# GenomicBreeding/GenomicBreedingModels.jl

Hardware: AMD Instinct MI355X
Metric: GRM+GBLUP genotype-cells/s (n x p) (higher is better)
Workload: dtype f64

## Files before the change

### genomicbreedingmodels.jl_amd/csrc/gbm_internal.h

```cpp
#pragma once
#include <hip/hip_runtime.h>
#include <stdint.h>
#include <functional>
#include <string>
#include <vector>

#include "../../include/gbm.h"

namespace gbm {

constexpr int64_t kNPadTile = 128;
constexpr int64_t kRhsRows = 64;
constexpr int kCholNB = 64;

inline int64_t round_up(int64_t x, int64_t m) { return (x + m - 1) / m * m; }
inline int64_t npad_of(int64_t n) { return round_up(n < 1 ? 1 : n, kNPadTile); }
inline int64_t gdim_of(int64_t n) { return npad_of(n) + kRhsRows; }

void set_error(const std::string& msg);
int fail(int code, const std::string& msg);
const std::string& last_error();

const char* knob(const char* name);
int64_t knob_i64(const char* name, int64_t def);

#define GBM_HIP_TRY(expr)                                                                      \
  do {                                                                                         \
    hipError_t e_ = (expr);                                                                    \
    if (e_ != hipSuccess)                                                                      \
      return ::gbm::fail(GBM_E_HIP, std::string("HIP error '") + hipGetErrorString(e_) +       \
                                        "' at " __FILE__ ":" + std::to_string(__LINE__) + " (" #expr ")"); \
  } while (0)

#define GBM_LAUNCH_CHECK() GBM_HIP_TRY(hipGetLastError())

#define GBM_TRY(expr)              \
  do {                             \
    int rc_ = (expr);              \
    if (rc_ != GBM_OK) return rc_; \
  } while (0)

int launch_grm(const double* Zt, int64_t ldz, int64_t p, int64_t n, double* G, int64_t ldg,
               void* ws, int64_t ws_bytes, hipStream_t s, int accum = 0, int32_t* err_out = nullptr);
bool grm_can_accumulate(int64_t n, int64_t p);
int launch_standardize_rows(const double* Xt, int64_t ldx, int64_t p, int64_t n, double* Zt, int64_t ldz, double* mean,
                            double* sd, int32_t* keep, int64_t* q_dev, hipStream_t s, bool beside_tiles = false);
bool standardize_fits_beside_tiles(int64_t n);
int64_t grm_workspace_bytes(int64_t n, int64_t p);
int launch_grm_export(const double* G, int64_t ldg, int64_t n, double inv_q, double* out, int64_t ldo, hipStream_t s);
int launch_predict(const double* Xt, int64_t ldx, int64_t p, int64_t n, const double* b, int64_t ldb, int64_t nrhs,
                   double* partial, int64_t nchunks, double* out, int64_t ldo, hipStream_t s);
int64_t predict_chunks(int64_t n, int64_t p);
int launch_add_inplace(double* a, const double* b, int64_t n, hipStream_t s);
int launch_standardize_i8(const int8_t* D, int64_t ldd, int64_t p, int64_t n, int ploidy, double* Zt, int64_t ldz,
                          double* mean, double* sd, int32_t* keep, int64_t* q_dev, hipStream_t s);
int launch_marker_rows(const double* Zt, int64_t ldz, int64_t p, int64_t n, const double* A, int64_t lda, int64_t nrhs,
                       double inv_q, const int64_t* q_dev, const double* sd, const int32_t* keep, double* B,
                       int64_t ldb, hipStream_t s);
int launch_marker_rows_i8(const int8_t* D, int64_t ldd, int64_t p, int64_t n, int ploidy, const double* A, int64_t lda,
                          int64_t nrhs, double inv_q, const int64_t* q_dev, const double* mean, const double* sd,
                          const int32_t* keep, double* B, int64_t ldb, hipStream_t s);
int launch_grm_exact(const int8_t* D, int64_t ldd, int64_t p, int64_t n, int ploidy, double* G, int64_t ldg,
                     double* mean, double* sd, int32_t* keep, int64_t* q_dev, int accum, void* ws, int64_t ws_bytes,
                     int32_t* slices_out, hipStream_t s);
int grm_exact_status(const void* ws, int64_t n, int64_t p, hipStream_t s);
int launch_gather_dosage(const double* Xt, int64_t ldx, int64_t p, const int32_t* idx, int64_t nT, int8_t* D,
                         hipStream_t s);
int launch_dosage_from_f64(const double* X, int64_t ldx, int64_t n, int64_t p, int8_t* D, int64_t ldd, int32_t* bad,
                           hipStream_t s);
// ... 79 lines not shown
```

### genomicbreedingmodels.jl_amd/csrc/grm.hip

```cpp
#include <algorithm>
#include <atomic>
#include <cmath>
#include <cstdio>
#include <cstdlib>
#include <map>
#include <mutex>
#include <queue>
#include <tuple>
#include <vector>

#include "chol_device.h"

namespace gbm {

constexpr int BT = 128;
constexpr int BK = 16;
constexpr int WPS = 2;
constexpr int LROW = BT + 2;
constexpr int STAGE = 2 * BK * LROW;

__device__ __forceinline__ void tile_of(int64_t t, int64_t& ti, int64_t& tj) {
  int64_t r = (int64_t)((sqrt(8.0 * (double)t + 1.0) - 1.0) * 0.5);
  while ((r + 1) * (r + 2) / 2 <= t) r++;
  while (r * (r + 1) / 2 > t) r--;
// ... 200 lines not shown
#pragma unroll
      for (int q = 0; q < ET; q++) b[st][q] = kv ? row[sb.e0 + q * 16 + fc] : 0.0;
    }
#pragma unroll
    for (int st = 0; st < 4; st++)
#pragma unroll
      for (int q = 0; q < ET; q++)
#pragma unroll
        for (int m = 0; m < 4; m++) acc[m][q] = __builtin_amdgcn_mfma_f64_16x16x4f64(a[st][m], b[st][q], acc[m][q], 0, 0, 0);
  }
  const int64_t rows = (int64_t)sb.erb * 256;
  constexpr int w = 16 * ET;
#pragma unroll
  for (int m = 0; m < 4; m++)
#pragma unroll
    for (int q = 0; q < ET; q++)
#pragma unroll
      for (int r = 0; r < 4; r++)
        part[((int64_t)ks * rows + i0 + m * 16 + fr + 4 * r) * w + q * 16 + fc] = acc[m][q][r];
}

template <int ET>
__global__ void __launch_bounds__(256, ET == 1 ? 4 : 1) grm_edge_kernel(const double* __restrict__ U, int64_t ldu, int64_t K,
                                                       SliceBounds sb, double* __restrict__ part) {
  grm_edge_pass<ET>(U, ldu, K, sb, blockIdx.x, part, threadIdx.x & 63, threadIdx.x >> 6);
}

__global__ void __launch_bounds__(256) grm_edge_reduce_kernel(const double* __restrict__ part, int64_t n,
                                                              SliceBounds sb, double* __restrict__ G, int64_t ldg,
                                                              int accum) {
  const int64_t idx = (int64_t)blockIdx.x * 256 + threadIdx.x;
  if (idx >= n * sb.er) return;
  const int64_t i = idx / sb.er;
  const int c = (int)(idx - i * sb.er);
  const int64_t rows = (int64_t)sb.erb * 256;
  const int w = 16 * sb.et;
  double acc = 0.0;
  for (int s = 0; s < sb.es; s++) acc += part[((int64_t)s * rows + i) * w + c];
  double* g = G + i * ldg + sb.e0 + c;
  *g = accum ? *g + acc : acc;
}

template <int MODE>
__global__ void __launch_bounds__(256, WPS)
syrk_kernel(const double* __restrict__ U, int64_t ldu, int64_t K, int64_t c0, int64_t lim,
            double* __restrict__ C, int64_t ldc, double* __restrict__ slab, int64_t ntiles, SliceBounds sb,
            double* __restrict__ Ld, double* __restrict__ Dinv, int32_t* __restrict__ info, int64_t fk0,
// ... 620 lines not shown
    const int64_t ti1 = (std::min(row_hi, gdim) - k1 + BT - 1) / BT;
    if (ti1 <= own.ti0) return GBM_OK;
    const int64_t m = ti1 - own.ti0;
    syrk_kernel<kSub><<<dim3((unsigned)m, (unsigned)(own.ncols + own.rhs)), 256, 0, s>>>(
        G + k0 * ldg, ldg, nb, k1, lim, G, ldg, nullptr, 0, SliceBounds{}, Ld, Dinv, info, -1, own);
    GBM_LAUNCH_CHECK();
    return GBM_OK;
  }
  if (nb == 64 && lim <= chol_small_lim()) {
    const int64_t m = (lim + 63) / 64;
    syrk64_sub_kernel<false><<<(unsigned)(m * (m + 1) / 2), 256, 0, s>>>(G + k0 * ldg, ldg, k1, lim, G, ldg, Ld, Dinv, info,
                                                                  next_k0, 0, (int)(nb / 64), ColKeep{});
    GBM_LAUNCH_CHECK();
    return GBM_OK;
  }
  const int64_t m = (lim + BT - 1) / BT;
  const int64_t ntiles = m * (m + 1) / 2;
  syrk_kernel<kSub><<<(unsigned)ntiles, 256, 0, s>>>(G + k0 * ldg, ldg, nb, k1, lim, G, ldg, nullptr, ntiles, SliceBounds{}, Ld,
                                                     Dinv, info, next_k0, own);
  GBM_LAUNCH_CHECK();
  return GBM_OK;
}

struct AuxStream {
  hipStream_t s = nullptr;
  hipEvent_t fork = nullptr, join = nullptr;
  ~AuxStream() {
    if (fork) (void)hipEventDestroy(fork);
    if (join) (void)hipEventDestroy(join);
  }
};
static int aux_stream(hipStream_t caller, AuxStream& a, bool* usable) {
  *usable = false;
  int dev = 0;
  GBM_HIP_TRY(hipGetDevice(&dev));
  if (caller) {
    int sdev = -1;
    if (hipStreamGetDevice(caller, &sdev) != hipSuccess) {
      (void)hipGetLastError();
      return GBM_OK;
    }
    if (sdev != dev) return GBM_OK;
  }
  static std::mutex mu;
  static std::map<int, hipStream_t> streams;
  {
    std::lock_guard<std::mutex> lock(mu);
    hipStream_t& hs = streams[dev];
    if (!hs) GBM_HIP_TRY(hipStreamCreateWithFlags(&hs, hipStreamNonBlocking));
    a.s = hs;
  }
  GBM_HIP_TRY(hipEventCreateWithFlags(&a.fork, hipEventDisableTiming));
  GBM_HIP_TRY(hipEventCreateWithFlags(&a.join, hipEventDisableTiming));
  *usable = true;
  return GBM_OK;
}

static int64_t grm_second_doubles(const GrmPlan& g) {
  return (g.persist && !g.sb.fuse && g.sb.n >= 2) ? g.tile_elems : 0;
}
static int64_t grm_counter_doubles(const GrmPlan& g) {
  return grm_second_doubles(g) + 4 + (g.sb.fuse ? (g.ntiles + 1) / 2 : 0);
}
int64_t grm_workspace_bytes(int64_t n, int64_t p) {
  const GrmPlan g = plan(n, p);
  return (g.main_doubles + g.edge_doubles + grm_counter_doubles(g)) * (int64_t)sizeof(double);
}

static int check_grm_args(const double* Zt, int64_t ldz, int64_t p, int64_t n, double* G, int64_t ldg) {
  const int64_t npad = npad_of(n);
  if (!Zt || !G || p < 1 || n < 1 || ldz < npad || ldg < npad || (ldz & 1) || (ldg & 1))
    return fail(GBM_E_ARG, "gbm_dev_grm: bad arguments (need ldz, ldg >= npad(n), both even)");
  if (((uintptr_t)Zt & 15) != 0 || ((uintptr_t)G & 15) != 0)
    return fail(GBM_E_ARG, "gbm_dev_grm: Zt and G must be 16-byte aligned");
  return GBM_OK;
}

static int launch_persist(const GrmPlan& g, SliceBounds sb, int s0, int cnt, const double* Zt, int64_t ldz, int64_t p,
                          int64_t lim, double* G, int64_t ldg, void* ws, int32_t* ctr, hipStream_t s) {
  sb.s0 = s0;
  sb.cnt = cnt;
  const int64_t units = (int64_t)cnt * g.ntiles;
  const unsigned pgrid = (unsigned)(units < resident_wgs() ? units : resident_wgs());
  if (g.sb.fuse)
    syrk_kernel<kPersistFused><<<pgrid, 256, 0, s>>>(Zt, ldz, p, 0, lim, G, ldg, (double*)ws, g.ntiles, sb, nullptr,
                                                     nullptr, ctr, -1, TileOwner{});
  else
    syrk_kernel<kPersist><<<pgrid, 256, 0, s>>>(Zt, ldz, p, 0, lim, G, ldg, (double*)ws, g.ntiles, sb, nullptr,
                                                nullptr, ctr, -1, TileOwner{});
  GBM_LAUNCH_CHECK();
  return GBM_OK;
}

static int launch_grm_edge(const GrmPlan& g, const double* Zt, int64_t ldz, int64_t p, int64_t n, double* G,
                           int64_t ldg, void* ws, int accum, hipStream_t es) {
  const unsigned eg = (unsigned)((int64_t)g.sb.erb * g.sb.es);
  double* part = (double*)ws + g.sb.eslab_off;
  switch (g.sb.et) {
    case 1: grm_edge_kernel<1><<<eg, 256, 0, es>>>(Zt, ldz, p, g.sb, part); break;
    case 2: grm_edge_kernel<2><<<eg, 256, 0, es>>>(Zt, ldz, p, g.sb, part); break;
    case 3: grm_edge_kernel<3><<<eg, 256, 0, es>>>(Zt, ldz, p, g.sb, part); break;
    default: grm_edge_kernel<4><<<eg, 256, 0, es>>>(Zt, ldz, p, g.sb, part); break;
  }
  GBM_LAUNCH_CHECK();
  if (g.edge_concurrent) {
    grm_edge_reduce_kernel<<<(unsigned)((n * g.sb.er + 255) / 256), 256, 0, es>>>(part, n, g.sb, G, ldg, accum);
    GBM_LAUNCH_CHECK();
  }
  return GBM_OK;
}

int launch_grm_syrk(const double* Zt, int64_t ldz, int64_t p, int64_t n, double* G, int64_t ldg, void* ws,
                    int64_t ws_bytes, hipStream_t s, int accum = 0) {
  int rc = check_grm_args(Zt, ldz, p, n, G, ldg);
  if (rc != GBM_OK) return rc;
  const GrmPlan g = plan(n, p);
  SliceBounds sb = g.sb;
  sb.accum = accum;
  const int64_t need = (g.main_doubles + g.edge_doubles + grm_counter_doubles(g)) * (int64_t)sizeof(double);
  if (need > 0 && (!ws || ws_bytes < need))
    return fail(GBM_E_ARG, "gbm_dev_grm: workspace too small (" + std::to_string(ws_bytes) + " < " +
                               std::to_string(need) + ")");
  const unsigned grid = (unsigned)(g.sb.n * ((g.ntiles + 7) & ~(int64_t)7));
  if (g.sb.carry) GBM_HIP_TRY(hipMemsetAsync(ws, 0, (size_t)(g.ntiles + 1) * sizeof(int32_t), s));
  int32_t* ctr = reinterpret_cast<int32_t*>((double*)ws + g.main_doubles + g.edge_doubles + grm_second_doubles(g));
// ... 10 lines not shown
      GBM_HIP_TRY(hipStreamWaitEvent(ax->s, ax->fork, 0));
    }
  }
  if (g.persist) {
    GBM_HIP_TRY(hipMemsetAsync(ctr, 0, (size_t)(8 + (g.sb.fuse ? g.ntiles : 0)) * sizeof(int32_t), s));
    rc = launch_persist(g, sb, 0, g.sb.n, Zt, ldz, p, lim, G, ldg, ws, ctr, s);
    if (rc != GBM_OK) return rc;
  } else {
    syrk_kernel<kSplit><<<grid, 256, 0, s>>>(Zt, ldz, p, 0, lim, G, ldg, (double*)ws, g.ntiles, sb, nullptr, nullptr,
                                             nullptr, -1, TileOwner{});
    GBM_LAUNCH_CHECK();
  }
  if (g.sb.er > 0) {
    rc = launch_grm_edge(g, Zt, ldz, p, n, G, ldg, ws, accum, ax ? ax->s : s);
    if (rc != GBM_OK) return rc;
    if (ax) {
      GBM_HIP_TRY(hipEventRecord(ax->join, ax->s));
      GBM_HIP_TRY(hipStreamWaitEvent(s, ax->join, 0));
    }
  }
  return GBM_OK;
}

int launch_standardize_grm_syrk(const double* X, int64_t ldx, int64_t p, int64_t n, double* Zt, int64_t ldz,
                                double* mean, double* sd, int32_t* keep, int64_t* q, double* G, int64_t ldg, void* ws,
                                int64_t ws_bytes, hipStream_t s) {
  int rc = check_grm_args(Zt, ldz, p, n, G, ldg);
  if (rc != GBM_OK) return rc;
  if (!X || !mean || !sd || !keep || !q || ldx < n || (X == Zt && ldx != ldz))
    return fail(GBM_E_ARG, "gbm_dev_standardize_grm_syrk: bad arguments");
  const GrmPlan g = plan(n, p);
  const int64_t h = g.sb.n >= 2 ? std::min<int64_t>(p, (int64_t)BK * g.sb.b[1]) : p;
  AuxStream aux;
  bool overlap = knob_i64("GBM_GRM_STD_OVERLAP", 1) != 0 && g.persist && !g.sb.fuse && g.sb.n >= 2 && h < p &&
                 standardize_fits_beside_tiles(n);
  if (overlap) {
    rc = aux_stream(s, aux, &overlap);
    if (rc != GBM_OK) return rc;
  }
  if (!overlap) {
    rc = launch_standardize_rows(X, ldx, p, n, Zt, ldz, mean, sd, keep, q, s);
    if (rc != GBM_OK) return rc;
    return launch_grm_syrk(Zt, ldz, p, n, G, ldg, ws, ws_bytes, s);
  }
  const int64_t need = (g.main_doubles + g.edge_doubles + grm_counter_doubles(g)) * (int64_t)sizeof(double);
  if (!ws || ws_bytes < need)
    return fail(GBM_E_ARG, "gbm_dev_standardize_grm_syrk: workspace too small (" + std::to_string(ws_bytes) + " < " +
                               std::to_string(need) + ")");
  int32_t* ctr = reinterpret_cast<int32_t*>((double*)ws + g.main_doubles + g.edge_doubles + grm_second_doubles(g)) - 8;
  const int64_t lim = g.sb.er > 0 ? g.sb.e0 : n;
  GBM_TRY(launch_standardize_rows(X, ldx, h, n, Zt, ldz, mean, sd, keep, q, s));
  GBM_HIP_TRY(hipMemsetAsync(ctr, 0, 16 * sizeof(int32_t), s));
  GBM_HIP_TRY(hipEventRecord(aux.fork, s));
  GBM_HIP_TRY(hipStreamWaitEvent(aux.s, aux.fork, 0));
  GBM_TRY(launch_persist(g, g.sb, 0, 1, Zt, ldz, p, lim, G, ldg, ws, ctr + 8, s));
  GBM_TRY(launch_standardize_rows(X + h * ldx, ldx, p - h, n, Zt + h * ldz, ldz, mean + h, sd + h, keep + h, q, aux.s,
                                  true));
  if (g.sb.er > 0) GBM_TRY(launch_grm_edge(g, Zt, ldz, p, n, G, ldg, ws, 0, aux.s));
  GBM_TRY(launch_persist(g, g.sb, 1, g.sb.n - 1, Zt, ldz, p, lim, G, ldg, ws, ctr, aux.s));
  GBM_HIP_TRY(hipEventRecord(aux.join, aux.s));
  GBM_HIP_TRY(hipStreamWaitEvent(s, aux.join, 0));
  return GBM_OK;
}

int launch_grm_reduce(int64_t n, int64_t p, double* G, int64_t ldg, const void* ws, hipStream_t s, int accum = 0,
                      int32_t* err_out = nullptr) {
  const GrmPlan g = plan(n, p);
  if (g.sb.n == 1 && g.sb.er == 0) return GBM_OK;
  if (!ws) return fail(GBM_E_ARG, "gbm_dev_grm_reduce: workspace required");
  if (g.sb.er > 0 && !g.edge_concurrent) {
    grm_edge_reduce_kernel<<<(unsigned)((n * g.sb.er + 255) / 256), 256, 0, s>>>((const double*)ws + g.sb.eslab_off, n,
                                                                                 g.sb, G, ldg, accum);
    GBM_LAUNCH_CHECK();
  }
  if (g.sb.n == 1 || g.sb.fuse) return GBM_OK;
  if (g.sb.carry && err_out) {
    GBM_HIP_TRY(hipMemcpyAsync(err_out, (const int32_t*)ws + g.ntiles, sizeof(int32_t), hipMemcpyDeviceToDevice, s));
    return GBM_OK;
  }
  if (g.sb.carry) {
    int32_t err = 0;
    GBM_HIP_TRY(hipMemcpyAsync(&err, (const int32_t*)ws + g.ntiles, sizeof(int32_t), hipMemcpyDeviceToHost, s));
    GBM_HIP_TRY(hipStreamSynchronize(s));
    if (err < 0)
// ... 75 lines not shown
}

extern "C" int gbm_dev_grm_syrk(const double* Zt, int64_t ldz, int64_t p, int64_t n, double* G, int64_t ldg,
                                void* workspace, int64_t ws_bytes, void* stream) {
  return gbm::launch_grm_syrk(Zt, ldz, p, n, G, ldg, workspace, ws_bytes, (hipStream_t)stream);
}

extern "C" int gbm_dev_standardize_grm_syrk(const double* Xt, int64_t ldx, int64_t p, int64_t n, double* Zt, int64_t ldz,
                                            double* mean, double* sd, int32_t* keep, int64_t* q_dev, double* G,
                                            int64_t ldg, void* workspace, int64_t ws_bytes, void* stream) {
  return gbm::launch_standardize_grm_syrk(Xt, ldx, p, n, Zt, ldz, mean, sd, keep, q_dev, G, ldg, workspace, ws_bytes,
                                          (hipStream_t)stream);
}

extern "C" int gbm_dev_grm_reduce(int64_t n, int64_t p, double* G, int64_t ldg, const void* workspace, void* stream) {
  if (!G || n < 1 || p < 1 || ldg < gbm::npad_of(n)) return gbm::fail(GBM_E_ARG, "gbm_dev_grm_reduce: bad arguments");
  return gbm::launch_grm_reduce(n, p, G, ldg, workspace, (hipStream_t)stream);
}

extern "C" int gbm_dev_grm_slices(int64_t n, int64_t p) {
  return gbm::plan(n, p).sb.n;
}

namespace gbm {
__global__ void __launch_bounds__(256) add_inplace_kernel(double* __restrict__ a, const double* __restrict__ b,
                                                          int64_t n) {
  for (int64_t i = ((int64_t)blockIdx.x * 256 + threadIdx.x) * 2; i < n; i += (int64_t)gridDim.x * 512) {
    if (i + 1 < n) {
      double2 x = *reinterpret_cast<const double2*>(a + i);
      const double2 y = *reinterpret_cast<const double2*>(b + i);
      x.x += y.x;
      x.y += y.y;
      *reinterpret_cast<double2*>(a + i) = x;
    } else {
      a[i] += b[i];
    }
  }
}

int launch_add_inplace(double* a, const double* b, int64_t n, hipStream_t s) {
  if (n <= 0) return GBM_OK;
  const int64_t want = (n + 511) / 512;
  add_inplace_kernel<<<(unsigned)(want < 8192 ? want : 8192), 256, 0, s>>>(a, b, n);
  GBM_LAUNCH_CHECK();
  return GBM_OK;
}
// ... 15 lines not shown
```

### genomicbreedingmodels.jl_amd/csrc/stats.hip

```cpp
#include <type_traits>

#include "counter_hash.h"
#include "gbm_internal.h"

namespace gbm {

__global__ void __launch_bounds__(256) synth_kernel(double* __restrict__ Xt, int64_t ldx, int64_t p,
                                                    int64_t n, uint64_t seed, int64_t j0) {
  for (int64_t j = blockIdx.y; j < p; j += gridDim.y) {
    const uint64_t base = mix64(seed * 0xD1B54A32D192ED03ull + (uint64_t)(j0 + j));
    const uint64_t thr = 214748364ull + (((base >> 32) * 1932735283ull) >> 32);
    double* row = Xt + j * ldx;
    for (int64_t i = (int64_t)blockIdx.x * 1024 + threadIdx.x; i < (int64_t)(blockIdx.x + 1) * 1024 && i < ldx;
         i += 256) {
      double v = 0.0;
      if (i < n) {
        const uint64_t h = mix64(base ^ ((uint64_t)i * 0x8CB92BA72F3D8DD7ull));
        const int d = ((h & 0xFFFFFFFFull) < thr) + ((h >> 32) < thr);
        v = 0.5 * (double)d;
      }
      row[i] = v;
    }
  }
}
// ... 43 lines not shown
  return (double)d * xs;
}

#ifndef GBM_STD_NT
#define GBM_STD_NT 1
#endif
template <typename T>
__device__ __forceinline__ double load_x(const T* row, int64_t i, double xs) {
  if constexpr (std::is_same<T, int8_t>::value)
    return dosage_x(row[i], xs);
  else if constexpr (GBM_STD_NT == 1 || GBM_STD_NT == 2)
    return __builtin_nontemporal_load(row + i);
  else
    return row[i];
}
__device__ __forceinline__ void store_z(double* z, double v) {
  if constexpr (GBM_STD_NT == 1 || GBM_STD_NT == 3)
    __builtin_nontemporal_store(v, z);
  else
    *z = v;
}

template <int BS, int NPT, bool GATHER, typename T>
__global__ void __launch_bounds__(BS) standardize_kernel(const T* Xt, int64_t ldx, int64_t p,
                                                         const int32_t* __restrict__ idx,
                                                         int64_t n, double* Zt, int64_t ldz,
                                                         double* __restrict__ mean,
                                                         double* __restrict__ sd, int32_t* __restrict__ keep,
                                                         unsigned long long* __restrict__ q_dev, int center_only,
                                                         double xs) {
  __shared__ double red[BS / 64];
  unsigned long long kept_local = 0;
  for (int64_t j = blockIdx.x; j < p; j += gridDim.x) {
    const T* row = Xt + j * ldx;
    double* zrow = Zt + j * ldz;
    double m, v;
    if constexpr (NPT > 0) {
      double x[NPT];
      double s = 0.0;
#pragma unroll
      for (int k = 0; k < NPT; k++) {
        const int64_t i = (int64_t)k * BS + threadIdx.x;
        x[k] = i < n ? load_x(row, GATHER ? idx[i] : i, xs) : 0.0;
        s += x[k];
      }
      m = block_sum<BS>(s, red) / (double)n;
      double ss = 0.0;
#pragma unroll
      for (int k = 0; k < NPT; k++) {
        const int64_t i = (int64_t)k * BS + threadIdx.x;
        const double d = x[k] - m;
        ss += i < n ? d * d : 0.0;
      }
// ... 16 lines not shown
    } else {
      double s = 0.0;
      for (int64_t i = threadIdx.x; i < n; i += BS) s += load_x(row, GATHER ? idx[i] : i, xs);
      m = block_sum<BS>(s, red) / (double)n;
      double ss = 0.0;
      for (int64_t i = threadIdx.x; i < n; i += BS) {
        const double d = load_x(row, GATHER ? idx[i] : i, xs) - m;
        ss += d * d;
      }
      v = n > 1 ? sqrt(block_sum<BS>(ss, red) / (double)(n - 1)) : __builtin_nan("");
      if (center_only) v = 1.0;
      const bool kp = (v > 2.220446049250313e-16) && isfinite(v);
      const double r = kp ? 1.0 / v : 0.0;
      for (int64_t i = threadIdx.x; i < ldz; i += BS) zrow[i] = (kp && i < n) ? (load_x(row, GATHER ? idx[i] : i, xs) - m) * r : 0.0;
      if (threadIdx.x == 0) {
        mean[j] = m;
        sd[j] = v;
        keep[j] = kp ? 1 : 0;
        kept_local += kp ? 1 : 0;
      }
    }
  }
  if (threadIdx.x == 0 && kept_local) atomicAdd(q_dev, kept_local);
}

template <int NPL, bool GATHER, typename T>
__global__ void __launch_bounds__(256) standardize_wave_kernel(const T* Xt, int64_t ldx, int64_t p,
                                                               const int32_t* __restrict__ idx, int64_t n,
                                                               double* Zt, int64_t ldz, double* __restrict__ mean,
                                                               double* __restrict__ sd, int32_t* __restrict__ keep,
                                                               unsigned long long* __restrict__ q_dev,
                                                               int center_only, double xs) {
  const int lane = threadIdx.x & 63;
  const int64_t w0 = (int64_t)blockIdx.x * 4 + (threadIdx.x >> 6), nw = (int64_t)gridDim.x * 4;
  unsigned long long kept_local = 0;
  for (int64_t j = w0; j < p; j += nw) {
    const T* row = Xt + j * ldx;
    double* zrow = Zt + j * ldz;
    double x[NPL];
    double s = 0.0;
#pragma unroll
    for (int k = 0; k < NPL; k++) {
      const int64_t i = (int64_t)k * 64 + lane;
      x[k] = i < n ? load_x(row, GATHER ? idx[i] : i, xs) : 0.0;
      s += x[k];
    }
// ... 90 lines not shown
    else GBM_STD_W(128);
#undef GBM_STD_W
    GBM_LAUNCH_CHECK();
    return GBM_OK;
  }
  if (n <= 256 * 4)
    standardize_kernel<256, 4, GATHER, T><<<grid, 256, 0, s>>>(Xt, ldx, p, idx, n, Zt, ldz, mean, sd, keep, q, center_only, xs);
  else if (n <= 256 * 8)
    standardize_kernel<256, 8, GATHER, T><<<grid, 256, 0, s>>>(Xt, ldx, p, idx, n, Zt, ldz, mean, sd, keep, q, center_only, xs);
  else if (n <= 256 * 16)
    standardize_kernel<256, 16, GATHER, T><<<grid, 256, 0, s>>>(Xt, ldx, p, idx, n, Zt, ldz, mean, sd, keep, q, center_only, xs);
  else if (n <= 256 * 32)
    standardize_kernel<256, 32, GATHER, T><<<grid, 256, 0, s>>>(Xt, ldx, p, idx, n, Zt, ldz, mean, sd, keep, q, center_only, xs);
  else
    standardize_kernel<256, 0, GATHER, T><<<grid, 256, 0, s>>>(Xt, ldx, p, idx, n, Zt, ldz, mean, sd, keep, q, center_only, xs);
  GBM_LAUNCH_CHECK();
  return GBM_OK;
}

namespace gbm {
bool standardize_fits_beside_tiles(int64_t n) { return n <= 256 * 20; }

int launch_standardize_rows(const double* Xt, int64_t ldx, int64_t p, int64_t n, double* Zt, int64_t ldz, double* mean,
                            double* sd, int32_t* keep, int64_t* q_dev, hipStream_t s, bool beside_tiles) {
  if (p == 0) return GBM_OK;
  if (beside_tiles && n > 256 * 16 && n <= 256 * 20) {
    standardize_kernel<256, 20, false, double><<<(unsigned)(p < 256 * 16 ? p : 256 * 16), 256, 0, s>>>(
        Xt, ldx, p, nullptr, n, Zt, ldz, mean, sd, keep, reinterpret_cast<unsigned long long*>(q_dev), 0, 1.0);
    GBM_LAUNCH_CHECK();
    return GBM_OK;
  }
  return launch_standardize<false>(Xt, ldx, p, nullptr, n, Zt, ldz, mean, sd, keep, q_dev, 0, s);
}

int launch_center_columns(const double* Xt, int64_t ldx, int64_t p, int64_t n, double* Zt, int64_t ldz, double* mean,
                          double* sd, int32_t* keep, int64_t* q_dev, hipStream_t s) {
  if (p == 0) return GBM_OK;
  return launch_standardize<false>(Xt, ldx, p, nullptr, n, Zt, ldz, mean, sd, keep, q_dev, 1, s);
}

int launch_standardize_i8(const int8_t* D, int64_t ldd, int64_t p, int64_t n, int ploidy, double* Zt, int64_t ldz,
                          double* mean, double* sd, int32_t* keep, int64_t* q_dev, hipStream_t s) {
  if (!D || !Zt || !mean || !sd || !keep || !q_dev || p < 0 || n < 1 || ldd < n || ldz < n || ploidy < 1)
    return fail(GBM_E_ARG, "standardize (int8 dosages): bad arguments");
  if (p == 0) return GBM_OK;
  return launch_standardize<false, int8_t>(D, ldd, p, nullptr, n, Zt, ldz, mean, sd, keep, q_dev, 0, s, 1.0 / ploidy);
}
}

extern "C" int gbm_dev_standardize(const double* Xt, int64_t ldx, int64_t p, int64_t n, double* Zt, int64_t ldz,
                                   double* mean, double* sd, int32_t* keep, int64_t* q_dev, void* stream) {
// ... 24 lines not shown
```

### genomicbreedingmodels.jl_amd/gbm/_lib.py

```python
from __future__ import annotations

import ctypes
import os
import threading

import numpy as np

ABI_VERSION = 212
GBM_OK = 0
GBM_E_ARG = -1
GBM_E_NOTPD = -2
GBM_E_HIP = -3
GBM_E_RCCL = -4
GBM_E_OOM = -5
GBM_E_NODEV = -6
GBM_E_DATA = -7

LIB_PATH = os.environ.get("GBM_LIBGBM") or os.path.join(os.path.dirname(os.path.abspath(__file__)), "libgbm.so")

EXPORTS = (
    "gbm_version", "gbm_last_error", "gbm_device_count", "gbm_device_allocations", "gbm_release_device_cache",
    "gbm_gblup_fit", "gbm_gblup_fit_reml", "gbm_gblup_fit_dosage_i8", "gbm_gblup_fit_synthetic", "gbm_grm", "gbm_grm_ploidy_aware", "gbm_colstats", "gbm_predict",
    "gbm_dev_npad", "gbm_dev_gdim", "gbm_dev_grm_workspace", "gbm_dev_solve_workspace",
    "gbm_dev_synth_genotypes", "gbm_dev_expand_dosage_i8", "gbm_dev_standardize", "gbm_dev_grm",
    "gbm_dev_grm_syrk", "gbm_dev_grm_reduce", "gbm_dev_grm_slices",
    "gbm_dev_gblup_solve", "gbm_dev_marker_effects",
    "gbm_dev_standardize_gather", "gbm_dev_gblup_terms",
    "gbm_session_create", "gbm_session_create_dosage_i8", "gbm_session_create_synthetic", "gbm_session_destroy", "gbm_session_gblup_fit",
    "gbm_session_predict", "gbm_session_reml_objective", "gbm_session_reml", "gbm_session_stats",
    "gbm_session_ridge_path", "gbm_session_ridge_lambda_max", "gbm_brr_fit", "gbm_bayes_fit",
    "gbm_dev_chol_prepare", "gbm_dev_chol_prepare_cols", "gbm_dev_chol_group_size", "gbm_dev_chol_group", "gbm_dev_chol_factor_diag",
    "gbm_dev_chol_strip_doubles", "gbm_dev_chol_strip_pack", "gbm_dev_chol_strip_unpack", "gbm_dev_chol_finish",
    "gbm_dev_grm_packed_size", "gbm_dev_grm_pack", "gbm_dev_grm_unpack",
    "gbm_debug_brr_stats", "gbm_debug_brr_shape", "gbm_debug_brr_trace", "gbm_debug_chol_flow_trace",
    "gbm_dev_synth_dosage_i8", "gbm_dev_standardize_i8", "gbm_dev_grm_accumulate", "gbm_dev_marker_effects_i8",
    "gbm_debug_oom_retries", "gbm_dev_chol_group_panels", "gbm_dev_chol_group_update", "gbm_dev_chol_strip_unpack_rows", "gbm_dev_chol_lower_copy",
    "gbm_dev_chol_area_doubles", "gbm_dev_chol_area_pack", "gbm_dev_chol_area_unpack",
    "gbm_dev_chol_group_update_cols", "gbm_dev_chol_group_update_tiles", "gbm_dev_grm_exact_workspace", "gbm_dev_grm_exact_i8",
    "gbm_gblup_fit_ex", "gbm_gblup_fit_reml_ex", "gbm_gblup_fit_dosage_i8_ex", "gbm_gblup_fit_synthetic_ex",
    "gbm_session_set_grm_mode", "gbm_session_grm_used", "gbm_debug_rccl_calls", "gbm_debug_xg_choose", "gbm_debug_chol_flow_order",
    "gbm_debug_chol_flow_order_check", "gbm_debug_chol_flow_order_size", "gbm_dev_grm_exact_status", "gbm_debug_set",
    "gbm_dev_whiten_rows", "gbm_session_gwas", "gbm_session_enet_path", "gbm_dev_standardize_grm_syrk",
    "gbm_dev_grm_symmetrize", "gbm_dev_rows_times_sym", "gbm_dev_rows_times_sym_workspace", "gbm_session_pcs",
    "gbm_debug_sym_eig",
)

GBM_GRM_DEFAULT, GBM_GRM_FP64, GBM_GRM_EXACT, GBM_GRM_AUTO, GBM_GRM_DROPIN = -1, 0, 1, 2, 3
GBM_PCS_GRM, GBM_PCS_REFERENCE = 0, 1
PCS_KINDS = {"grm": GBM_PCS_GRM, "reference": GBM_PCS_REFERENCE}
GRM_MODES = {None: GBM_GRM_DEFAULT, "default": GBM_GRM_DEFAULT, "fp64": GBM_GRM_FP64, "exact": GBM_GRM_EXACT,
             "auto": GBM_GRM_AUTO, "dropin": GBM_GRM_DROPIN}


def grm_mode(mode) -> int:
    if isinstance(mode, int) and mode in GRM_MODES.values():
        return mode
    try:
        return GRM_MODES[mode]
    except (KeyError, TypeError):
        raise ArgumentError(f"grm must be one of 'auto', 'exact', 'fp64', 'dropin' or None, got {mode!r}") from None


class ArgumentError(ValueError):
    """Mirrors Julia's ArgumentError thrown by the reference (e.g. src/prediction.jl:67-112)."""


class GBMError(RuntimeError):
# ... 165 lines not shown
    lib.gbm_debug_xg_choose.argtypes = [D, D, P, P]
    lib.gbm_debug_chol_flow_order.restype = I64
    lib.gbm_debug_chol_flow_order.argtypes = [I32, P, I64]
    lib.gbm_debug_chol_flow_order_size.restype = I64
    lib.gbm_debug_chol_flow_order_size.argtypes = [I32]
    lib.gbm_debug_chol_flow_order_check.restype = I64
    lib.gbm_debug_chol_flow_order_check.argtypes = [I32, P, I64]
    lib.gbm_dev_grm_exact_status.restype = I32
    lib.gbm_dev_grm_exact_status.argtypes = [P, I64, I64, P]
    lib.gbm_dev_whiten_rows.restype = I32
    lib.gbm_dev_whiten_rows.argtypes = [P, I64, I64, P, P, I64, I64, P]
    lib.gbm_session_gwas.restype = I32
    lib.gbm_session_gwas.argtypes = [P, P, I64, P, P, I64, I64, I32, D, D, P, P, P, P]
    lib.gbm_dev_grm_symmetrize.restype = I32
    lib.gbm_dev_grm_symmetrize.argtypes = [P, I64, I64, D, P, I64, P]
    lib.gbm_dev_rows_times_sym_workspace.restype = I64
    lib.gbm_dev_rows_times_sym_workspace.argtypes = [I64, I64]
    lib.gbm_dev_rows_times_sym.restype = I32
    lib.gbm_dev_rows_times_sym.argtypes = [P, I64, I64, P, I64, I64, P, I64, P, I64, P]
    lib.gbm_session_pcs.restype = I32
    lib.gbm_session_pcs.argtypes = [P, P, I64, I32, I64, D, I64, P, P, P, P, P]
    lib.gbm_debug_sym_eig.restype = I32
    lib.gbm_debug_sym_eig.argtypes = [P, I32, P, P]
    lib.gbm_debug_set.restype = I32
    lib.gbm_debug_set.argtypes = [ctypes.c_char_p, ctypes.c_char_p]
    return lib


def _bind_runtime_first():
    if os.environ.get("GBM_NO_TORCH") == "1":
        return
    try:
        import torch
    except ImportError:
        return


def load():
    global _lib
    with _lock:
        if _lib is None:
            if not os.path.exists(LIB_PATH):
                raise ImportError(
                    f"libgbm.so not found at {LIB_PATH}: build it with `python -c 'import __graft_entry__ as g; g.build()'`"
                    " (the GBLUP path has no CPU fallback)")
            _bind_runtime_first()
# ... 44 lines not shown
```

### include/gbm.h

```cpp
#ifndef GBM_H
#define GBM_H

#include <stdint.h>

#ifdef __cplusplus
extern "C" {
#endif

#define GBM_VERSION 212

#define GBM_OK 0
#define GBM_E_ARG (-1)
#define GBM_E_NOTPD (-2)
#define GBM_E_HIP (-3)
#define GBM_E_RCCL (-4)
#define GBM_E_OOM (-5)
#define GBM_E_NODEV (-6)
#define GBM_E_DATA (-7)

#define GBM_GRM_DEFAULT (-1)
#define GBM_GRM_FP64 0
#define GBM_GRM_EXACT 1
#define GBM_GRM_AUTO 2
#define GBM_GRM_DROPIN 3
// ... 217 lines not shown
                int64_t n_burnin, int64_t thin, double r2, double df0, uint64_t seed, int device,
                double* b_hat_out, double* y_pred_out, double* var_out);

#define GBM_BAYES_A 1
#define GBM_BAYES_B 2
#define GBM_BAYES_C 3
int gbm_bayes_fit(int model, const double* X, int64_t n, int64_t p, int64_t ldx, const double* y,
                  int64_t n_iter, int64_t n_burnin, int64_t thin, double r2, double df0, double prob_in,
                  double counts, uint64_t seed, int device, double* b_hat_out ,
                  double* y_pred_out , double* var_out ,
                  double* pip_out );

int gbm_debug_brr_stats(int* last_path, int64_t* fallbacks);
int gbm_debug_brr_shape(int* C, int* O, int* R, int* Ko, int* Kn);
int gbm_debug_oom_retries(int64_t* retries, int64_t* contexts_freed);
int64_t gbm_debug_brr_trace(int64_t* host, int64_t cap);
int64_t gbm_debug_chol_flow_trace(int64_t* host, int64_t cap);
int64_t gbm_debug_chol_flow_order(int nbc, int32_t* order_out, int64_t cap);
int64_t gbm_debug_chol_flow_order_size(int nbc);
int64_t gbm_debug_chol_flow_order_check(int nbc, const int32_t* order, int64_t m);
int gbm_debug_rccl_calls(int64_t* allreduce, int64_t* allgather);
int gbm_debug_xg_choose(double wmin, double wmax, int* slices_out, int* shift_out);
int gbm_debug_set(const char* name, const char* value);

int gbm_debug_sym_eig(const double* A, int m, double* w, double* V);
#ifdef __cplusplus
}
#endif

#endif
```

Measured before the change: 12.15 billion.

## Add multi-launch front schedule overlapping standardization with GRM persistent slices

Adds a scheduler that splits the standardize-then-SYRK front into several slice launches. A simulated slot model picks the split so that standardizing each row chunk on an aux stream finishes before the persistent GRM tiles need it. A second aux stream, preallocated per-device events, and an optional wave priority (s_setprio) for the helper kernels are added. By default (GBM_GRM_FRONT=0) it keeps the old two-launch path, now using cached events and a per-device mutex instead of per-call event creation. It also adds NPT-specialized beside-tile standardize kernels, which are only used when priority is set or n is above 4096.

```diff
diff --git a/genomicbreedingmodels.jl_amd/csrc/gbm_internal.h b/genomicbreedingmodels.jl_amd/csrc/gbm_internal.h
--- a/genomicbreedingmodels.jl_amd/csrc/gbm_internal.h
+++ b/genomicbreedingmodels.jl_amd/csrc/gbm_internal.h
@@ -40,11 +40,23 @@
     if (rc_ != GBM_OK) return rc_; \
   } while (0)
 
+#ifdef __HIPCC__
+__device__ __forceinline__ void set_helper_prio(int prio) {
+  switch (prio) {
+    case 1: __builtin_amdgcn_s_setprio(1); break;
+    case 2: __builtin_amdgcn_s_setprio(2); break;
+    case 3: __builtin_amdgcn_s_setprio(3); break;
+    default: break;
+  }
+}
+#endif
+
 int launch_grm(const double* Zt, int64_t ldz, int64_t p, int64_t n, double* G, int64_t ldg,
                void* ws, int64_t ws_bytes, hipStream_t s, int accum = 0, int32_t* err_out = nullptr);
 bool grm_can_accumulate(int64_t n, int64_t p);
 int launch_standardize_rows(const double* Xt, int64_t ldx, int64_t p, int64_t n, double* Zt, int64_t ldz, double* mean,
-                            double* sd, int32_t* keep, int64_t* q_dev, hipStream_t s, bool beside_tiles = false);
+                            double* sd, int32_t* keep, int64_t* q_dev, hipStream_t s, bool beside_tiles = false,
+                            int prio = 0);
 bool standardize_fits_beside_tiles(int64_t n);
 int64_t grm_workspace_bytes(int64_t n, int64_t p);
 int launch_grm_export(const double* G, int64_t ldg, int64_t n, double inv_q, double* out, int64_t ldo, hipStream_t s);
diff --git a/genomicbreedingmodels.jl_amd/csrc/grm.hip b/genomicbreedingmodels.jl_amd/csrc/grm.hip
--- a/genomicbreedingmodels.jl_amd/csrc/grm.hip
+++ b/genomicbreedingmodels.jl_amd/csrc/grm.hip
@@ -246,7 +246,8 @@
 
 template <int ET>
 __global__ void __launch_bounds__(256, ET == 1 ? 4 : 1) grm_edge_kernel(const double* __restrict__ U, int64_t ldu, int64_t K,
-                                                       SliceBounds sb, double* __restrict__ part) {
+                                                       SliceBounds sb, double* __restrict__ part, int prio) {
+  set_helper_prio(prio);
   grm_edge_pass<ET>(U, ldu, K, sb, blockIdx.x, part, threadIdx.x & 63, threadIdx.x >> 6);
 }
 
@@ -913,15 +914,23 @@
   return GBM_OK;
 }
 
+constexpr int kMaxFrontLaunches = 16;
+struct DeviceAux {
+  std::mutex mu;
+  hipStream_t s = nullptr, s2 = nullptr;
+  hipEvent_t fork = nullptr, join = nullptr, join2 = nullptr;
+  hipEvent_t chunk[kMaxFrontLaunches] = {};
+};
 struct AuxStream {
   hipStream_t s = nullptr;
   hipEvent_t fork = nullptr, join = nullptr;
+  DeviceAux* dev = nullptr;
   ~AuxStream() {
     if (fork) (void)hipEventDestroy(fork);
     if (join) (void)hipEventDestroy(join);
   }
 };
-static int aux_stream(hipStream_t caller, AuxStream& a, bool* usable) {
+static int aux_stream(hipStream_t caller, AuxStream& a, bool* usable, bool per_call_events = true) {
   *usable = false;
   int dev = 0;
   GBM_HIP_TRY(hipGetDevice(&dev));
@@ -934,15 +943,26 @@
     if (sdev != dev) return GBM_OK;
   }
   static std::mutex mu;
-  static std::map<int, hipStream_t> streams;
+  static std::map<int, DeviceAux*> sets;
   {
     std::lock_guard<std::mutex> lock(mu);
-    hipStream_t& hs = streams[dev];
-    if (!hs) GBM_HIP_TRY(hipStreamCreateWithFlags(&hs, hipStreamNonBlocking));
-    a.s = hs;
-  }
-  GBM_HIP_TRY(hipEventCreateWithFlags(&a.fork, hipEventDisableTiming));
-  GBM_HIP_TRY(hipEventCreateWithFlags(&a.join, hipEventDisableTiming));
+    DeviceAux*& d = sets[dev];
+    if (!d) d = new DeviceAux();
+    if (!d->s) GBM_HIP_TRY(hipStreamCreateWithFlags(&d->s, hipStreamNonBlocking));
+    if (!per_call_events && !d->chunk[kMaxFrontLaunches - 1]) {
+      if (!d->s2) GBM_HIP_TRY(hipStreamCreateWithFlags(&d->s2, hipStreamNonBlocking));
+      for (hipEvent_t* e : {&d->fork, &d->join, &d->join2})
+        if (!*e) GBM_HIP_TRY(hipEventCreateWithFlags(e, hipEventDisableTiming));
+      for (int i = 0; i < kMaxFrontLaunches; i++)
+        if (!d->chunk[i]) GBM_HIP_TRY(hipEventCreateWithFlags(&d->chunk[i], hipEventDisableTiming));
+    }
+    a.s = d->s;
+    a.dev = d;
+  }
+  if (per_call_events) {
+    GBM_HIP_TRY(hipEventCreateWithFlags(&a.fork, hipEventDisableTiming));
+    GBM_HIP_TRY(hipEventCreateWithFlags(&a.join, hipEventDisableTiming));
+  }
   *usable = true;
   return GBM_OK;
 }
@@ -984,14 +1004,14 @@
 }
 
 static int launch_grm_edge(const GrmPlan& g, const double* Zt, int64_t ldz, int64_t p, int64_t n, double* G,
-                           int64_t ldg, void* ws, int accum, hipStream_t es) {
+                           int64_t ldg, void* ws, int accum, hipStream_t es, int prio = 0) {
   const unsigned eg = (unsigned)((int64_t)g.sb.erb * g.sb.es);
   double* part = (double*)ws + g.sb.eslab_off;
   switch (g.sb.et) {
-    case 1: grm_edge_kernel<1><<<eg, 256, 0, es>>>(Zt, ldz, p, g.sb, part); break;
-    case 2: grm_edge_kernel<2><<<eg, 256, 0, es>>>(Zt, ldz, p, g.sb, part); break;
-    case 3: grm_edge_kernel<3><<<eg, 256, 0, es>>>(Zt, ldz, p, g.sb, part); break;
-    default: grm_edge_kernel<4><<<eg, 256, 0, es>>>(Zt, ldz, p, g.sb, part); break;
+    case 1: grm_edge_kernel<1><<<eg, 256, 0, es>>>(Zt, ldz, p, g.sb, part, prio); break;
+    case 2: grm_edge_kernel<2><<<eg, 256, 0, es>>>(Zt, ldz, p, g.sb, part, prio); break;
+    case 3: grm_edge_kernel<3><<<eg, 256, 0, es>>>(Zt, ldz, p, g.sb, part, prio); break;
+    default: grm_edge_kernel<4><<<eg, 256, 0, es>>>(Zt, ldz, p, g.sb, part, prio); break;
   }
   GBM_LAUNCH_CHECK();
   if (g.edge_concurrent) {
@@ -1048,6 +1068,136 @@
   return GBM_OK;
 }
 
+#ifndef GBM_GRM_FRONT_DEFAULT
+#define GBM_GRM_FRONT_DEFAULT 0
+#endif
+struct FrontLaunch {
+  int32_t s0, cnt;
+  int64_t r0, r1;
+};
+
+constexpr double kStdAloneValuesPerUs = 74.0 * 5000.0;
+constexpr double kStdBesideValuesPerUs = 8.7 * 5000.0;
+constexpr double kFrontSafety = 1.25;
+constexpr double kFrontStageUs = 3.9;
+
+static int64_t front_row(const GrmPlan& g, int64_t p, int s) { return std::min<int64_t>(p, (int64_t)BK * g.sb.b[s]); }
+
+static bool front_from_starts(const GrmPlan& g, int64_t p, const std::vector<int>& starts, std::vector<FrontLaunch>& out) {
+  const int S = g.sb.n;
+  out.clear();
+  if (starts.empty() || (int)starts.size() > kMaxFrontLaunches - 2) return false;
+  std::vector<int> sorted(starts);
+  std::sort(sorted.begin(), sorted.end());
+  for (size_t i = 0; i < sorted.size(); i++)
+    if (sorted[i] < 0 || sorted[i] >= S || (i > 0 && sorted[i] == sorted[i - 1])) return false;
+  auto add = [&](int s0, int s1) { out.push_back({s0, s1 - s0, front_row(g, p, s0), front_row(g, p, s1)}); };
+  for (int st : starts) {
+    auto it = std::upper_bound(sorted.begin(), sorted.end(), st);
+    add(st, it == sorted.end() ? st + 1 : *it);
+  }
+  if (sorted.front() > 0) add(0, sorted.front());
+  if (sorted.back() + 1 < S) add(sorted.back() + 1, S);
+  return true;
+}
+
+static std::vector<double> front_first_slot(const GrmPlan& g, const std::vector<FrontLaunch>& ls,
+                                            const std::vector<double>& cost, int64_t R) {
+  std::vector<double> speed(R);
+  uint64_t h = 0x9E3779B97F4A7C15ull;
+  for (int64_t k = 0; k < R; k++) {
+    h = h * 6364136223846793005ull + 1442695040888963407ull;
+    speed[k] = 1.0 + 0.035 * (((double)(h >> 11) / 9007199254740992.0) * 2.0 - 1.0);
+  }
+  std::priority_queue<std::pair<double, int64_t>, std::vector<std::pair<double, int64_t>>, std::greater<>> slots;
+  for (int64_t k = 0; k < R; k++) slots.push({0.0, k});
+  std::vector<double> first;
+  for (const FrontLaunch& l : ls) {
+    first.push_back(slots.top().first);
+    for (int sl = l.s0; sl < l.s0 + l.cnt; sl++)
+      for (double c : cost) {
+        auto [f, k] = slots.top();
+        slots.pop();
+        slots.push({f + (double)(g.sb.b[sl + 1] - g.sb.b[sl]) * c / speed[k], k});
+      }
+  }
+  return first;
+}
+
+static bool front_applies(const GrmPlan& g, int64_t n, int64_t p) {
+  return knob_i64("GBM_GRM_STD_OVERLAP", 1) != 0 && g.persist && !g.sb.fuse && g.sb.n >= 2 &&
+         front_row(g, p, 1) < p && standardize_fits_beside_tiles(n);
+}
+
+static std::vector<FrontLaunch> front_schedule(const GrmPlan& g, int64_t n, int64_t p, bool* two_launch = nullptr) {
+  std::vector<FrontLaunch> best;
+  const int S = g.sb.n;
+  if (two_launch) *two_launch = false;
+  if (const char* ov = ::gbm::knob("GBM_GRM_FRONT_ORDER")) {
+    std::vector<int> starts;
+    bool ok = *ov != 0;
+    for (const char* q = ov; ok && *q;) {
+      char* end = nullptr;
+      const long x = strtol(q, &end, 10);
+      if (end == q) ok = false;
+      starts.push_back((int)x);
+      q = (*end == ',') ? end + 1 : end;
+      if (*end != ',' && *end != 0) ok = false;
+    }
+    if (ok && front_from_starts(g, p, starts, best)) return best;
+  }
+  front_from_starts(g, p, {0}, best);
+  if (knob_i64("GBM_GRM_FRONT", GBM_GRM_FRONT_DEFAULT) == 0) {
+    if (two_launch) *two_launch = true;
+    return best;
+  }
+  if (S < 3) return best;
+  const int64_t R = resident_wgs();
+  static std::mutex mu;
+  static std::map<std::tuple<int64_t, int64_t, int64_t, std::vector<int32_t>, double>, std::vector<int>> cache;
+  const GrmTuning tune = grm_tuning();
+  auto key = std::make_tuple(n, p, R * 4096 + g.ntiles, std::vector<int32_t>(g.sb.b, g.sb.b + S + 1), tune.diag_cost);
+  std::vector<int> starts;
+  {
+    std::lock_guard<std::mutex> lock(mu);
+    auto it = cache.find(key);
+    if (it != cache.end()) starts = it->second;
+  }
+  if (starts.empty()) {
+    std::vector<double> cost;
+    for (int64_t tj = 0; (int64_t)cost.size() < g.ntiles; tj++)
+      for (int64_t ti = 0; ti <= tj; ti++) cost.push_back(ti == tj ? tune.diag_cost : 1.0);
+    std::vector<std::vector<int>> cands;
+    for (int k = 1; k + 1 < S; k++) cands.push_back({k, 0});
+    for (int k2 = 2; k2 + 1 < S; k2++)
+      for (int k1 = 1; k1 < k2; k1++) cands.push_back({k2, k1, 0});
+    starts = {0};
+    int64_t exposed = best[0].r1 - best[0].r0;
+    size_t launches = best.size();
+    std::vector<FrontLaunch> ls;
+    for (const auto& c : cands) {
+      if (!front_from_starts(g, p, c, ls)) continue;
+      const int64_t rows0 = ls[0].r1 - ls[0].r0;
+      if (rows0 > exposed || (rows0 == exposed && ls.size() >= launches)) continue;
+      const std::vector<double> first = front_first_slot(g, ls, cost, R);
+      double ready = (double)rows0 * (double)n / kStdAloneValuesPerUs;
+      bool ok = true;
+      for (size_t i = 1; i < ls.size() && ok; i++) {
+        ready += (double)(ls[i].r1 - ls[i].r0) * (double)n / kStdBesideValuesPerUs;
+        ok = ready * kFrontSafety <= first[i] * kFrontStageUs;
+      }
+      if (!ok) continue;
+      starts = c;
+      exposed = rows0;
+      launches = ls.size();
+    }
+    std::lock_guard<std::mutex> lock(mu);
+    cache.emplace(key, starts);
+  }
+  front_from_starts(g, p, starts, best);
+  return best;
+}
+
 int launch_standardize_grm_syrk(const double* X, int64_t ldx, int64_t p, int64_t n, double* Zt, int64_t ldz,
                                 double* mean, double* sd, int32_t* keep, int64_t* q, double* G, int64_t ldg, void* ws,
                                 int64_t ws_bytes, hipStream_t s) {
@@ -1056,12 +1206,10 @@
   if (!X || !mean || !sd || !keep || !q || ldx < n || (X == Zt && ldx != ldz))
     return fail(GBM_E_ARG, "gbm_dev_standardize_grm_syrk: bad arguments");
   const GrmPlan g = plan(n, p);
-  const int64_t h = g.sb.n >= 2 ? std::min<int64_t>(p, (int64_t)BK * g.sb.b[1]) : p;
   AuxStream aux;
-  bool overlap = knob_i64("GBM_GRM_STD_OVERLAP", 1) != 0 && g.persist && !g.sb.fuse && g.sb.n >= 2 && h < p &&
-                 standardize_fits_beside_tiles(n);
+  bool overlap = front_applies(g, n, p);
   if (overlap) {
-    rc = aux_stream(s, aux, &overlap);
+    rc = aux_stream(s, aux, &overlap, false);
     if (rc != GBM_OK) return rc;
   }
   if (!overlap) {
@@ -1073,19 +1221,43 @@
   if (!ws || ws_bytes < need)
     return fail(GBM_E_ARG, "gbm_dev_standardize_grm_syrk: workspace too small (" + std::to_string(ws_bytes) + " < " +
                                std::to_string(need) + ")");
-  int32_t* ctr = reinterpret_cast<int32_t*>((double*)ws + g.main_doubles + g.edge_doubles + grm_second_doubles(g)) - 8;
+  bool two_launch = false;
+  const std::vector<FrontLaunch> ls = front_schedule(g, n, p, &two_launch);
+  const int L = (int)ls.size();
+  const int prio = (int)std::min<int64_t>(3, std::max<int64_t>(0, knob_i64("GBM_GRM_HELPER_PRIO", 0)));
+  int32_t* tail = reinterpret_cast<int32_t*>((double*)ws + g.main_doubles + g.edge_doubles + grm_second_doubles(g));
   const int64_t lim = g.sb.er > 0 ? g.sb.e0 : n;
-  GBM_TRY(launch_standardize_rows(X, ldx, h, n, Zt, ldz, mean, sd, keep, q, s));
-  GBM_HIP_TRY(hipMemsetAsync(ctr, 0, 16 * sizeof(int32_t), s));
-  GBM_HIP_TRY(hipEventRecord(aux.fork, s));
-  GBM_HIP_TRY(hipStreamWaitEvent(aux.s, aux.fork, 0));
-  GBM_TRY(launch_persist(g, g.sb, 0, 1, Zt, ldz, p, lim, G, ldg, ws, ctr + 8, s));
-  GBM_TRY(launch_standardize_rows(X + h * ldx, ldx, p - h, n, Zt + h * ldz, ldz, mean + h, sd + h, keep + h, q, aux.s,
-                                  true));
-  if (g.sb.er > 0) GBM_TRY(launch_grm_edge(g, Zt, ldz, p, n, G, ldg, ws, 0, aux.s));
-  GBM_TRY(launch_persist(g, g.sb, 1, g.sb.n - 1, Zt, ldz, p, lim, G, ldg, ws, ctr, aux.s));
-  GBM_HIP_TRY(hipEventRecord(aux.join, aux.s));
-  GBM_HIP_TRY(hipStreamWaitEvent(s, aux.join, 0));
+  DeviceAux& d = *aux.dev;
+  std::lock_guard<std::mutex> lock(d.mu);
+  auto chunk = [&](const FrontLaunch& l, hipStream_t st, bool beside) {
+    return launch_standardize_rows(X + l.r0 * ldx, ldx, l.r1 - l.r0, n, Zt + l.r0 * ldz, ldz, mean + l.r0, sd + l.r0,
+                                   keep + l.r0, q, st, beside, beside ? prio : 0);
+  };
+  GBM_TRY(chunk(ls[0], s, false));
+  GBM_HIP_TRY(hipMemsetAsync(tail - 8 * (L - 1), 0, (size_t)(8 * L) * sizeof(int32_t), s));
+  GBM_HIP_TRY(hipEventRecord(d.fork, s));
+  GBM_HIP_TRY(hipStreamWaitEvent(d.s, d.fork, 0));
+  GBM_TRY(launch_persist(g, g.sb, ls[0].s0, ls[0].cnt, Zt, ldz, p, lim, G, ldg, ws, tail, s));
+  if (two_launch) {
+    GBM_TRY(chunk(ls[1], d.s, true));
+    if (g.sb.er > 0) GBM_TRY(launch_grm_edge(g, Zt, ldz, p, n, G, ldg, ws, 0, d.s, prio));
+    GBM_TRY(launch_persist(g, g.sb, ls[1].s0, ls[1].cnt, Zt, ldz, p, lim, G, ldg, ws, tail - 8, d.s));
+    GBM_HIP_TRY(hipEventRecord(d.join, d.s));
+    GBM_HIP_TRY(hipStreamWaitEvent(s, d.join, 0));
+    return GBM_OK;
+  }
+  for (int i = 1; i < L; i++) {
+    GBM_TRY(chunk(ls[i], d.s, true));
+    GBM_HIP_TRY(hipEventRecord(d.chunk[i], d.s));
+    const hipStream_t ts = (i & 1) ? d.s2 : s;
+    GBM_HIP_TRY(hipStreamWaitEvent(ts, d.chunk[i], 0));
+    GBM_TRY(launch_persist(g, g.sb, ls[i].s0, ls[i].cnt, Zt, ldz, p, lim, G, ldg, ws, tail - 8 * i, ts));
+  }
+  if (g.sb.er > 0) GBM_TRY(launch_grm_edge(g, Zt, ldz, p, n, G, ldg, ws, 0, d.s, prio));
+  GBM_HIP_TRY(hipEventRecord(d.join, d.s));
+  GBM_HIP_TRY(hipEventRecord(d.join2, d.s2));
+  GBM_HIP_TRY(hipStreamWaitEvent(s, d.join2, 0));
+  GBM_HIP_TRY(hipStreamWaitEvent(s, d.join, 0));
   return GBM_OK;
 }
 
@@ -1207,6 +1379,20 @@
   return gbm::plan(n, p).sb.n;
 }
 
+extern "C" int64_t gbm_debug_grm_front_schedule(int64_t n, int64_t p, int64_t* out, int64_t cap) {
+  if (n < 1 || p < 1) return 0;
+  const gbm::GrmPlan g = gbm::plan(n, p);
+  if (!gbm::front_applies(g, n, p)) return 0;
+  const std::vector<gbm::FrontLaunch> ls = gbm::front_schedule(g, n, p);
+  for (int64_t i = 0; out && i < (int64_t)ls.size() && i < cap; i++) {
+    out[4 * i] = ls[i].s0;
+    out[4 * i + 1] = ls[i].cnt;
+    out[4 * i + 2] = ls[i].r0;
+    out[4 * i + 3] = ls[i].r1;
+  }
+  return (int64_t)ls.size();
+}
+
 namespace gbm {
 __global__ void __launch_bounds__(256) add_inplace_kernel(double* __restrict__ a, const double* __restrict__ b,
                                                           int64_t n) {
diff --git a/genomicbreedingmodels.jl_amd/csrc/stats.hip b/genomicbreedingmodels.jl_amd/csrc/stats.hip
--- a/genomicbreedingmodels.jl_amd/csrc/stats.hip
+++ b/genomicbreedingmodels.jl_amd/csrc/stats.hip
@@ -89,13 +89,13 @@
 }
 
 template <int BS, int NPT, bool GATHER, typename T>
-__global__ void __launch_bounds__(BS) standardize_kernel(const T* Xt, int64_t ldx, int64_t p,
-                                                         const int32_t* __restrict__ idx,
-                                                         int64_t n, double* Zt, int64_t ldz,
-                                                         double* __restrict__ mean,
-                                                         double* __restrict__ sd, int32_t* __restrict__ keep,
-                                                         unsigned long long* __restrict__ q_dev, int center_only,
-                                                         double xs) {
+__device__ __forceinline__ void standardize_rows(const T* Xt, int64_t ldx, int64_t p,
+                                                 const int32_t* __restrict__ idx,
+                                                 int64_t n, double* Zt, int64_t ldz,
+                                                 double* __restrict__ mean,
+                                                 double* __restrict__ sd, int32_t* __restrict__ keep,
+                                                 unsigned long long* __restrict__ q_dev, int center_only,
+                                                 double xs) {
   __shared__ double red[BS / 64];
   unsigned long long kept_local = 0;
   for (int64_t j = blockIdx.x; j < p; j += gridDim.x) {
@@ -158,6 +158,26 @@
     }
   }
   if (threadIdx.x == 0 && kept_local) atomicAdd(q_dev, kept_local);
+}
+
+template <int BS, int NPT, bool GATHER, typename T>
+__global__ void __launch_bounds__(BS) standardize_kernel(const T* Xt, int64_t ldx, int64_t p,
+                                                         const int32_t* __restrict__ idx,
+                                                         int64_t n, double* Zt, int64_t ldz,
+                                                         double* __restrict__ mean,
+                                                         double* __restrict__ sd, int32_t* __restrict__ keep,
+                                                         unsigned long long* __restrict__ q_dev, int center_only,
+                                                         double xs) {
+  standardize_rows<BS, NPT, GATHER, T>(Xt, ldx, p, idx, n, Zt, ldz, mean, sd, keep, q_dev, center_only, xs);
+}
+
+template <int NPT>
+__global__ void __launch_bounds__(256) standardize_beside_kernel(const double* Xt, int64_t ldx, int64_t p, int64_t n,
+                                                                 double* Zt, int64_t ldz, double* __restrict__ mean,
+                                                                 double* __restrict__ sd, int32_t* __restrict__ keep,
+                                                                 unsigned long long* __restrict__ q_dev, int prio) {
+  set_helper_prio(prio);
+  standardize_rows<256, NPT, false, double>(Xt, ldx, p, nullptr, n, Zt, ldz, mean, sd, keep, q_dev, 0, 1.0);
 }
 
 template <int NPL, bool GATHER, typename T>
@@ -294,11 +314,17 @@
 bool standardize_fits_beside_tiles(int64_t n) { return n <= 256 * 20; }
 
 int launch_standardize_rows(const double* Xt, int64_t ldx, int64_t p, int64_t n, double* Zt, int64_t ldz, double* mean,
-                            double* sd, int32_t* keep, int64_t* q_dev, hipStream_t s, bool beside_tiles) {
-  if (p == 0) return GBM_OK;
-  if (beside_tiles && n > 256 * 16 && n <= 256 * 20) {
-    standardize_kernel<256, 20, false, double><<<(unsigned)(p < 256 * 16 ? p : 256 * 16), 256, 0, s>>>(
-        Xt, ldx, p, nullptr, n, Zt, ldz, mean, sd, keep, reinterpret_cast<unsigned long long*>(q_dev), 0, 1.0);
+                            double* sd, int32_t* keep, int64_t* q_dev, hipStream_t s, bool beside_tiles, int prio) {
+  if (p == 0) return GBM_OK;
+  if (beside_tiles && n <= 256 * 20 && (n > 256 * 16 || prio > 0)) {
+    const unsigned grid = (unsigned)(p < 256 * 16 ? p : 256 * 16);
+    auto q = reinterpret_cast<unsigned long long*>(q_dev);
+#define GBM_STD_B(NPT) standardize_beside_kernel<NPT><<<grid, 256, 0, s>>>(Xt, ldx, p, n, Zt, ldz, mean, sd, keep, q, prio)
+    if (n <= 256 * 4) GBM_STD_B(4);
+    else if (n <= 256 * 8) GBM_STD_B(8);
+    else if (n <= 256 * 16) GBM_STD_B(16);
+    else GBM_STD_B(20);
+#undef GBM_STD_B
     GBM_LAUNCH_CHECK();
     return GBM_OK;
   }
diff --git a/genomicbreedingmodels.jl_amd/gbm/_lib.py b/genomicbreedingmodels.jl_amd/gbm/_lib.py
--- a/genomicbreedingmodels.jl_amd/gbm/_lib.py
+++ b/genomicbreedingmodels.jl_amd/gbm/_lib.py
@@ -42,7 +42,7 @@
     "gbm_debug_chol_flow_order_check", "gbm_debug_chol_flow_order_size", "gbm_dev_grm_exact_status", "gbm_debug_set",
     "gbm_dev_whiten_rows", "gbm_session_gwas", "gbm_session_enet_path", "gbm_dev_standardize_grm_syrk",
     "gbm_dev_grm_symmetrize", "gbm_dev_rows_times_sym", "gbm_dev_rows_times_sym_workspace", "gbm_session_pcs",
-    "gbm_debug_sym_eig",
+    "gbm_debug_sym_eig", "gbm_debug_grm_front_schedule",
 )
 
 GBM_GRM_DEFAULT, GBM_GRM_FP64, GBM_GRM_EXACT, GBM_GRM_AUTO, GBM_GRM_DROPIN = -1, 0, 1, 2, 3
@@ -254,6 +254,8 @@
     lib.gbm_session_pcs.argtypes = [P, P, I64, I32, I64, D, I64, P, P, P, P, P]
     lib.gbm_debug_sym_eig.restype = I32
     lib.gbm_debug_sym_eig.argtypes = [P, I32, P, P]
+    lib.gbm_debug_grm_front_schedule.restype = I64
+    lib.gbm_debug_grm_front_schedule.argtypes = [I64, I64, P, I64]
     lib.gbm_debug_set.restype = I32
     lib.gbm_debug_set.argtypes = [ctypes.c_char_p, ctypes.c_char_p]
     return lib
diff --git a/include/gbm.h b/include/gbm.h
--- a/include/gbm.h
+++ b/include/gbm.h
@@ -263,6 +263,7 @@
 int gbm_debug_rccl_calls(int64_t* allreduce, int64_t* allgather);
 int gbm_debug_xg_choose(double wmin, double wmax, int* slices_out, int* shift_out);
 int gbm_debug_set(const char* name, const char* value);
+int64_t gbm_debug_grm_front_schedule(int64_t n, int64_t p, int64_t* out, int64_t cap);
 
 int gbm_debug_sym_eig(const double* A, int m, double* w, double* V);
 #ifdef __cplusplus
```

Result: no change. 12.13 billion (-0.1%).
